# sbelharbi/sr-caco-2

Measured on AMD Instinct MI355X. Metric: train patches/sec, SwinIR x8 64->512 1ch, higher is better.
Workload: dtype f32 (fp16x2 split-MFMA, f32 accumulate)

## Files before the change

### include/srhip.h

```cpp
#ifndef SRHIP_H
#define SRHIP_H
#ifdef __cplusplus
extern "C" {
#endif
#if defined(__GNUC__) || defined(__clang__)
#pragma GCC visibility push(default)
#endif

const char* srhip_last_error(void);
int srhip_abi_version(void);
int srhip_experiments_enabled(void);
int srhip_set_matmul_mode(int mode);
int srhip_get_matmul_mode(void);


int srhip_gemm_nt(const float* A, long lda, const float* W, long ldw, const float* bias, float* C,
                  long ldc, int M, int N, int K, int a_mode, const float* ln_stats, int epi,
                  const float* R, long ldr, const float* rowscale, int rows_per_scale, float alpha,
                  float* aux, long ldaux, void* stream);

int srhip_gemm_nt_batched(const float* A, long lda, long a_z0, long a_z1, const float* W, long ldw, long w_z0, long w_z1, float* C,
                          long ldc, long c_z0, long c_z1, int M, int N, int K, int zcount, int zdiv, void* stream);

int srhip_conv3x3_nhwc(const float* X, long ldx, const float* Wp, const float* bias, float* Y, long ldy,
// ... 115 lines not shown
  float* part;
  float* part_colsum;
} srhip_tn_problem;
int srhip_tn_tiles(int NI, int NJ);
int srhip_tn_group_plan(int M, int ntiles, int* S);
int srhip_gemm_tn_grouped(const srhip_tn_problem* probs, int nprob, int M, int S, void* stream);
int srhip_conv3x3_wgrad(const float* dY, long lddy, const float* X, long ldx, int B, int H, int W,
                        int Cout, int Cin, float* part, float* part_colsum, int S, void* stream);

int srhip_tn_plan_bx3(int M, int NI, int NJ, int conv, int* S, long* part_floats);
int srhip_tn_group_plan_bx3(int M, int ntiles, int* S);
int srhip_gemm_tn_bx3(const float* A, long lda, const float* B, long ldb, int M, int NI, int NJ,
                      const float* a_rowscale, int a_rowscale_rows, int b_mode, const float* ln_stats,
                      float* part, float* part_colsum, int S, void* stream);
int srhip_gemm_tn_grouped_bx3(const srhip_tn_problem* probs, int nprob, int M, int S, void* stream);
int srhip_conv3x3_wgrad_bx3(const float* dY, long lddy, const float* X, long ldx, int B, int H, int W,
                            int Cout, int Cin, float* part, float* part_colsum, int S, void* stream);
int srhip_reduce_linear_wgrad(const float* part, const float* colsum, int S, float* dW, float* db,
                              int N, int K, void* stream);
long srhip_ln_affine_ws(int N, int K);
int srhip_reduce_ln_linear_wgrad(const float* part, const float* colsum, int S, const float* W,
                                 const float* gamma, const float* beta, float* dW, float* db,
                                 float* dgamma, float* dbeta, int N, int K, float* ln_ws,
                                 void* stream);
typedef struct {
  const float* part; const float* colsum;
  const float* W; const float* gamma; const float* beta;
  float* dW; float* db; float* dgamma; float* dbeta;
  int N, K;
  float* ln_ws;
} srhip_reduce_problem;
int srhip_reduce_wgrad_grouped(const srhip_reduce_problem* probs, int nprob, int S, void* stream);
int srhip_reduce_conv_wgrad(const float* part, const float* colsum, int S, float* dW, float* db,
                            int Co, int Ci, void* stream);

int srhip_fold_layernorm(const float* W, const float* b, const float* gamma, const float* beta,
                         float* Wf, float* bf, int N, int K, void* stream);
int srhip_transpose(const float* in, float* out, int R, int C, void* stream);
int srhip_pack_conv_weight(const float* w, float* wp, float* wpt, int Co, int Ci, void* stream);

int srhip_layernorm_fwd(const float* x, float* stats, float* y, const float* gamma, const float* beta,
                        long M, int C, void* stream);
long srhip_layernorm_bwd_ws(long M, int C);
int srhip_layernorm_bwd(const float* dy, const float* x, const float* stats, const float* res,
                        const float* gamma, float* out, float* dgamma, float* dbeta, float* workspace, long M,
                        int C, void* stream);

// ... 215 lines not shown
```

### sr-caco-2_amd/csrc/api.hip

```cpp
#include <stdarg.h>
#include "common.h"
#include "kernels.h"
#include "../../include/srhip.h"

static thread_local char g_err[512] = "";

int sr_fail(int code, const char* fmt, ...) {
  va_list ap;
  va_start(ap, fmt);
  vsnprintf(g_err, sizeof(g_err), fmt, ap);
  va_end(ap);
  return code;
}

extern "C" {

const char* srhip_last_error(void) { return g_err; }
int srhip_abi_version(void) { return 13; }
int srhip_experiments_enabled(void) {
#ifdef SRHIP_EXPERIMENTS
  return 1;
#else
  return 0;
#endif
// ... 357 lines not shown
}
int srhip_gemm_tn_bx3(const float* A, long lda, const float* B, long ldb, int M, int NI, int NJ,
                      const float* a_rowscale, int a_rowscale_rows, int b_mode, const float* ln_stats,
                      float* part, float* part_colsum, int S, void* stream) {
  return gemm_tn_any(true, A, lda, B, ldb, M, NI, NJ, a_rowscale, a_rowscale_rows, b_mode, ln_stats, part,
                     part_colsum, S, stream);
}

int srhip_tn_tiles(int NI, int NJ) { return sr_tn_tiles(NI, NJ); }
int srhip_tn_plan_bx3(int M, int NI, int NJ, int conv, int* S, long* part_floats) {
  return sr_tn_plan_bx3(M, NI, NJ, conv, S, part_floats);
}
int srhip_tn_group_plan_bx3(int M, int ntiles, int* S) { return sr_tn_group_plan_t(M, ntiles, 256, S); }
int srhip_tn_group_plan(int M, int ntiles, int* S) { return sr_tn_group_plan(M, ntiles, S); }

static int gemm_tn_grouped_any(bool bx, const srhip_tn_problem* probs, int nprob, int M, int S, void* stream) {
  SR_REQUIRE(nprob >= 1 && nprob <= (bx ? 24 : 4), "gemm_tn_grouped: 1..%d problems", bx ? 24 : 4);
  TnArgs a[24];
  memset(a, 0, sizeof(a));
  for (int k = 0; k < nprob; ++k) {
    const srhip_tn_problem& q = probs[k];
    SR_REQUIRE(q.b_mode >= 0 && q.b_mode <= 2, "gemm_tn_grouped: b_mode %d", q.b_mode);
    SR_REQUIRE(q.b_mode != 1 || q.ln_stats, "gemm_tn_grouped: layernorm prologue without stats");
    TnArgs& p = a[k];
    p.A = q.A; p.lda = q.lda; p.B = q.B; p.ldb = q.ldb; p.M = M; p.NI = q.NI; p.NJ = q.NJ;
    p.a_rowscale = q.a_rowscale; p.a_rowscale_rows = q.a_rowscale_rows; p.b_mode = q.b_mode;
    p.ln_stats = q.ln_stats; p.part = q.part; p.part_colsum = q.part_colsum; p.S = S;
  }
  return bx ? sr_gemm_tnb_grouped(a, nprob, (hipStream_t)stream) : sr_gemm_tn_grouped(a, nprob, (hipStream_t)stream);
}
int srhip_gemm_tn_grouped(const srhip_tn_problem* probs, int nprob, int M, int S, void* stream) {
  return gemm_tn_grouped_any(false, probs, nprob, M, S, stream);
}
int srhip_gemm_tn_grouped_bx3(const srhip_tn_problem* probs, int nprob, int M, int S, void* stream) {
  return gemm_tn_grouped_any(true, probs, nprob, M, S, stream);
}

static int conv3x3_ps2_split(int wfmt, const float* X, long ldx, const void* Wb, const float* bias, float* Yup, long ldy,
                          int B, int H, int W, int Cin, int Cout, int epi, float alpha, void* stream) {
  SR_REQUIRE(epi == 0 || epi == 1 || epi == 6, "conv3x3_ps2_bx3: epi %d (0 bias | 1 relu | 6 leaky relu)", epi);
  NtArgs p;
  memset(&p, 0, sizeof(p));
  p.A = X; p.lda = ldx; p.Wb = (const unsigned short*)Wb; p.C = Yup; p.ldc = ldy;
  p.N = Cout; p.K = Cin; p.bias = bias; p.epi = epi; p.rows_per_scale = H * W; p.alpha = alpha;
  p.batch = B; p.H = H; p.Wd = W; p.ps = 1; p.wfmt = wfmt;
  return sr_conv3x3_ntb(p, (hipStream_t)stream);
}
static int conv3x3_ps2_bwd_data_split(int wfmt, const float* dYup, long lddy, const void* Wbt, float* dX, long ldx, int B, int H,
                                   int W, int Cout, int Cin, int epi, const float* R, long ldr, float alpha,
                                   void* stream) {
// ... 56 lines not shown
```

### sr-caco-2_amd/csrc/gemm_tnb.hip

```cpp
#include <stdlib.h>
#include "common.h"
#include "kernels.h"

typedef __bf16 bf16x8 __attribute__((ext_vector_type(8)));
typedef __bf16 bf16x2 __attribute__((ext_vector_type(2)));
typedef float f32x2 __attribute__((ext_vector_type(2)));
typedef unsigned u32x4 __attribute__((ext_vector_type(4)));

namespace {

constexpr int TKB = 32;

__device__ const float k_tnb_zero_row[256] = {0.f};

__device__ __forceinline__ f32x16 mfma_bf(u32x4 a, u32x4 b, f32x16 c) {
  return __builtin_amdgcn_mfma_f32_32x32x16_bf16(__builtin_bit_cast(bf16x8, a),
                                                 __builtin_bit_cast(bf16x8, b), c, 0, 0, 0);
}

typedef _Float16 f16x8 __attribute__((ext_vector_type(8)));
typedef _Float16 tn_f16x2 __attribute__((ext_vector_type(2)));
__device__ __forceinline__ f32x16 mfma_h(u32x4 a, u32x4 b, f32x16 c) {
  return __builtin_amdgcn_mfma_f32_32x32x16_f16(__builtin_bit_cast(f16x8, a), __builtin_bit_cast(f16x8, b), c, 0, 0, 0);
}
// ... 315 lines not shown

  if (do_colsum) {
    float* red = (float*)smem;
    if (producer && !isB) {
#pragma unroll
      for (int j = 0; j < W; ++j) red[hh * BC + W * lane + j] = cs[j];
    }
    __syncthreads();
    if (tid < ivalid) {
      const int io = i0 + tid;
      p.part_colsum[(long)s * p.NI + (p.ps ? (io % ps_f) * 4 + io / ps_f : io)] = red[tid] + red[BC + tid];
    }
  }
}

template <int W, int BM = -1, bool AR = false, bool NR = false, bool CONV = false>
__device__ __forceinline__ void tnb_body_h(const TnArgs& p, const int s, const int tile, unsigned char* smem, const int tap = 0) {
  const int bmode = BM >= 0 ? BM : p.b_mode;
  const bool arow = BM >= 0 ? AR : (p.a_rowscale != nullptr);
  constexpr int BC = 64 * W, HC = 32 * W;
  constexpr int PLANE = 2 * BC * 64;
  constexpr int BUF = 3 * PLANE;
  constexpr int CTRL = 2 * PLANE;
  constexpr int SINV = 2 * PLANE + 4096;

  const int tid = threadIdx.x, lane = tid & 63;
  const int wave8 = __builtin_amdgcn_readfirstlane(tid >> 6);
  const bool producer = wave8 >= 4;
  const int wave = wave8 & 3;
  const int wi = wave >> 1, wj = wave & 1, r = lane & 31, h = lane >> 5;
  const int nbj = (p.NJ + p.j_tile - 1) / p.j_tile;
  const int bi = tile / nbj, bj = tile - bi * nbj;
  const int i0 = bi * p.i_tile, j0 = bj * p.j_tile;
  const int ivalid = min(p.i_tile, p.NI - i0), jvalid = min(p.j_tile, p.NJ - j0);
  const int m_begin = s * p.rows_per_slice;
  const int m_end = min(p.M, m_begin + p.rows_per_slice);
  const bool do_colsum = p.part_colsum && bj == 0 && tap == 0;
  const int cdy = CONV ? tap / 3 - 1 : 0, cdx = CONV ? tap % 3 - 1 : 0;

  struct Stage {
    typename ColVec<W>::T rv[2][8];
    float scale;
    float2 stats;
    int trow;
  };
  Stage sg0, sg1;
  const bool isB = wave & 1;
  const int ch = wave >> 1;
  const int lt = lane & 31, th = lane >> 5;
  const int opvalid = isB ? jvalid : ivalid;
  const int gcol = HC * ch + W * lt;
  const int colq = max(min(gcol, opvalid - W), 0);
  const int dsh = gcol - colq;
// ... 294 lines not shown
#pragma unroll
        for (int q = 0; q < 16; ++q) {
          const int row = (wi * W + i) * 32 + mfma_row(q, lane);
          if (row < ivalid) out[(long)(i0 + row) * p.NJ + j0 + col] = acc[i][j][q] * (sinv[row] * ib);
        }
      }
  }

  if (do_colsum) {
    float* red = (float*)smem;
    if (producer && !isB) {
#pragma unroll
      for (int j = 0; j < W; ++j) red[th * BC + gcol + j] = cs[j];
    }
    __syncthreads();
    if (tid < ivalid) p.part_colsum[(long)s * p.NI + i0 + tid] = red[tid] + red[BC + tid];
  }
}

constexpr int TK9 = 16;
__device__ __forceinline__ int unit_slot9(int col, int u) { return 2 * col + (u ^ ((col >> 3) & 1)); }
constexpr int T9_OPS = 6;
constexpr int T9_PLANE = T9_OPS * 64 * 32;
constexpr int T9_CTRL = 2 * T9_PLANE;
constexpr int T9_BUF = 2 * T9_PLANE + 2048;
constexpr int T9_SINV = 2 * T9_BUF;
constexpr int T9_LDS = 2 * T9_BUF + 2048;
constexpr int T9_THREADS = 14 * 64;

template <int H2, int DBG = 0>
// ... 513 lines not shown

template <int W>
__global__ void __launch_bounds__(512, 1) k_tnb_hc(TnArgs p, int tiles, int xcd) {
  extern __shared__ __attribute__((aligned(16))) unsigned char smem[];
  const int L = xcd ? sr_xcd_block(blockIdx.x, gridDim.x) : (int)blockIdx.x;
  const int tap = L % 9, t2 = L / 9;
  const bool even = p.NI % W == 0 && p.NJ % W == 0 && p.i_tile % W == 0 && p.j_tile % W == 0;
  if (even) tnb_body_h<W, 0, false, true, true>(p, t2 / tiles, t2 % tiles, smem, tap);
  else tnb_body_h<W, 0, false, false, true>(p, t2 / tiles, t2 % tiles, smem, tap);
}

constexpr int TNB_GROUP_MAX = 24;
struct TnbGroup {
  TnArgs p[TNB_GROUP_MAX];
  int tile_start[TNB_GROUP_MAX + 1];
  int n, S, xcd;
};
__device__ __forceinline__ void tnb_group_block(const TnbGroup& g, int& slice, int& t) {
  const int tiles = g.tile_start[g.n];
  if (g.xcd) {
    const int L = sr_xcd_block(blockIdx.x, gridDim.x);
    t = L % tiles;
    slice = L / tiles;
  } else {
    slice = blockIdx.x % g.S;
    t = blockIdx.x / g.S;
  }
}
template <int W>
__global__ void __launch_bounds__(512, 1) k_tnb_grouped(TnbGroup g) {
  extern __shared__ __attribute__((aligned(16))) unsigned char smem[];
  int slice, t;
  tnb_group_block(g, slice, t);
  TnArgs p = g.p[0];
  int t0 = 0;
#pragma unroll
  for (int i = 1; i < TNB_GROUP_MAX; ++i)
    if (i < g.n && t >= g.tile_start[i]) { p = g.p[i]; t0 = g.tile_start[i]; }
  tnb_body<W>(p, slice, t - t0, 0, smem);
}

template <int W>
__global__ void __launch_bounds__(512, 1) k_tnb_grouped_h(TnbGroup g) {
  extern __shared__ __attribute__((aligned(16))) unsigned char smem[];
  int slice, t;
  tnb_group_block(g, slice, t);
  TnArgs p = g.p[0];
  int t0 = 0;
#pragma unroll
  for (int i = 1; i < TNB_GROUP_MAX; ++i)
    if (i < g.n && t >= g.tile_start[i]) { p = g.p[i]; t0 = g.tile_start[i]; }
  const bool even = p.NI % W == 0 && p.NJ % W == 0 && p.i_tile % W == 0 && p.j_tile % W == 0;
  if (even && p.b_mode == 1 && !p.a_rowscale) tnb_body_h<W, 1, false, true>(p, slice, t - t0, smem);
  else if (even && p.b_mode == 0 && p.a_rowscale) tnb_body_h<W, 0, true, true>(p, slice, t - t0, smem);
  else if (even && p.b_mode == 2 && p.a_rowscale) tnb_body_h<W, 2, true, true>(p, slice, t - t0, smem);
  else tnb_body_h<W>(p, slice, t - t0, smem);
}

constexpr int TNB_BATCH_MAX = 40;
struct TnbConvBatch {
  TnArgs base;
  const float* A[TNB_BATCH_MAX];
  const float* B[TNB_BATCH_MAX];
  long part_stride, colsum_stride;
  int n, tiles, xcd;
};
template <int W>
__global__ void __launch_bounds__(512, 1) k_tnb_conv_batched(TnbConvBatch g) {
  extern __shared__ __attribute__((aligned(16))) unsigned char smem[];
  const int L = g.xcd ? sr_xcd_block(blockIdx.x, gridDim.x) : (int)blockIdx.x;
  const int tap = L % 9;
// ... 102 lines not shown
  if (e != hipSuccess) return sr_fail(-5, "%s: cannot reserve %d B of LDS: %s", name, bytes, hipGetErrorString(e));
  return 0;
}

constexpr int lds_bytes(int w) { return 2 * 3 * 2 * 64 * w * 64; }
constexpr long TNB_W1_SLOTS = 3 * 256;

}

int sr_gemm_tnb_grouped(TnArgs* probs, int n, hipStream_t st) {
  SR_REQUIRE(n >= 1 && n <= TNB_GROUP_MAX, "gemm_tn_grouped_bx3: 1..%d problems (got %d)", TNB_GROUP_MAX, n);
  static_assert(sizeof(TnbGroup) <= 4096, "kernel arguments");
  TnbGroup g;
  memset(&g, 0, sizeof(g));
  g.n = n;
  int w = 1, tiles = 0;
  for (int k = 0; k < n; ++k) {
    TnArgs& p = probs[k];
    SR_REQUIRE(p.M == probs[0].M && p.S == probs[0].S && !p.conv,
               "gemm_tn_grouped_bx3: problems must share M and S");
    SR_REQUIRE(p.NI % 4 == 0 && p.NJ % 4 == 0 && p.lda % 4 == 0 && p.ldb % 4 == 0,
               "gemm_tn_grouped_bx3: NI, NJ, lda, ldb must be multiples of 4");
    int a, b;
    p.i_tile = pick_tile(p.NI, &a);
    p.j_tile = pick_tile(p.NJ, &b);
    if (a > w) w = a;
    if (b > w) w = b;
    const int rps = sr_cdiv(p.M, p.S);
    p.rows_per_slice = (rps + TKB - 1) / TKB * TKB;
    g.tile_start[k] = tiles;
    tiles += sr_cdiv(p.NI, p.i_tile) * sr_cdiv(p.NJ, p.j_tile);
    g.p[k] = p;
  }
  g.tile_start[n] = tiles;
  g.S = probs[0].S;
  static const int gxcd = [] { const char* e = sr_getenv("SRHIP_TN_GROUP_XCD"); return e ? atoi(e) : 1; }();
  g.xcd = gxcd;
  dim3 grid(probs[0].S * tiles, 1, 1);
  static bool attr[4] = {false, false, false, false};
#define SR_TNB_G(W_)                                                                      \
  if (w == W_) {                                                                          \
    if (!attr[W_]) {                                                                      \
      if (int rc = reserve_lds(k_tnb_grouped<W_>, lds_bytes(W_), "k_tnb_grouped")) return rc; \
      attr[W_] = true;                                                                    \
    }                                                                                     \
    hipLaunchKernelGGL((k_tnb_grouped<W_>), grid, dim3(512), lds_bytes(W_), st, g);       \
  }
  if (w == 3) {
    static bool attr_h = false;
    if (!attr_h) {
      if (int rc = reserve_lds(k_tnb_grouped_h<3>, lds_bytes(3), "k_tnb_grouped_h")) return rc;
      attr_h = true;
    }
    hipLaunchKernelGGL((k_tnb_grouped_h<3>), grid, dim3(512), lds_bytes(3), st, g);
  }
  SR_TNB_G(1) SR_TNB_G(2)
#undef SR_TNB_G
  SR_LAUNCH_CHECK("k_tnb_grouped");
  return 0;
}

int sr_gemm_tnb(TnArgs& p, hipStream_t st) {
  SR_REQUIRE(p.M > 0 && p.S > 0, "gemm_tn_bx3: empty problem");
  SR_REQUIRE(p.NI % 4 == 0 && p.NJ % 4 == 0 && p.lda % 4 == 0 && p.ldb % 4 == 0,
             "gemm_tn_bx3: NI, NJ, lda, ldb must be multiples of 4");
  int tile;
  const int w = pick_w(p.NI, p.NJ, &tile);
  p.i_tile = p.j_tile = tile;
  SR_REQUIRE(!p.ps || (p.conv && p.NI % 4 == 0 && (p.NI / 4) % w == 0 && p.NI % p.i_tile == 0),
             "conv3x3_wgrad + PixelShuffle(2): Cout/4 = %d must be a multiple of %d (columns per lane), Cout of the tile", p.NI / 4, w);
  const int rps = sr_cdiv(p.M, p.S);
  p.rows_per_slice = (rps + TKB - 1) / TKB * TKB;
  int tiles = sr_cdiv(p.NI, p.i_tile) * sr_cdiv(p.NJ, p.j_tile);
// ... 174 lines not shown
```

### sr-caco-2_amd/csrc/kernels.h

```cpp
#pragma once
#include <hip/hip_runtime.h>

struct NtArgs {
  const float* A; long lda;
  const float* W; long ldw; long wtap;
  float* C; long ldc;
  int M, N, K;
  int n_tile;
  int xcd_order;
  const float* bias;
  int a_mode;
  const float* ln_stats;
  int epi;
  const float* slope;
  const float* pro_coef;
  const float* R; long ldr;
  float* aux; long ldaux;
  const float* R2; long ldr2; const float* ep_stats;
  int wide_epi;
  float* stats_out;
  const float* rowscale; int rows_per_scale; float alpha;
  int batch, H, Wd, tiles_x, tiles_y;
  int dbg;
  int stagger;
// ... 114 lines not shown
int sr_prep_table(const PrepEntry* tab_dev, int n, int total_blocks, hipStream_t st);
__host__ __device__ static inline int sr_kp(int K) { return (K + 31) / 32 * 32; }
int sr_split3(const float* W, long ldw, int rows, int K, unsigned short* out, hipStream_t st);
int sr_gemm_ntb(NtArgs& p, hipStream_t st);
int sr_conv3x3_ntb(NtArgs& p, hipStream_t st);
int sr_gemm_ntb_lnbwd(NtArgs& p, hipStream_t st);
int sr_gemm_ntp(NtArgs& p, hipStream_t st);
int sr_gemm_ntw(NtArgs& p, hipStream_t st);
int sr_conv3x3_ntcw(NtArgs& p, hipStream_t st);
int sr_conv3x3_ntcw2(NtArgs& p, int rows_per_wave, hipStream_t st);
int sr_conv3x3_nhcw(NtArgs& p, hipStream_t st);
int sr_conv3x3_nhcw2(NtArgs& p, int rows_per_wave, hipStream_t st);
int sr_gemm_tn(TnArgs& p, hipStream_t st);
int sr_gemm_tnb(TnArgs& p, hipStream_t st);
int sr_gemm_tnb_grouped(TnArgs* probs, int n, hipStream_t st);
int sr_tn_plan(int M, int NI, int NJ, int conv, int* S, long* part_floats);
int sr_gemm_tn_grouped(TnArgs* probs, int n, hipStream_t st);
int sr_tn_group_plan(int M, int ntiles, int* S);
int sr_tn_plan_t(int M, int NI, int NJ, int conv, int target, int* S, long* part_floats);
int sr_tn_plan_bx3(int M, int NI, int NJ, int conv, int* S, long* part_floats);
int sr_tn_group_plan_t(int M, int ntiles, int dflt_target, int* S);
int sr_tn_tiles(int NI, int NJ);
int sr_conv_wgrad_batched_plan(int n, int M, int NI, int NJ, int* S, long* part_floats_per_item);
int sr_conv_wgrad_batched_tnb(const TnArgs& base, const float* const* A, const float* const* B, int n,
                              long part_stride, long colsum_stride, hipStream_t st);
```

### sr-caco-2_amd/csrc/misc.hip

```cpp
#include "common.h"
#include "kernels.h"
#include "../../include/srhip.h"

namespace {

__global__ void k_reduce_slices(const float* __restrict__ part, float* __restrict__ out,
                                long n, int S, float beta, const float* __restrict__ colsum,
                                float* __restrict__ db, int nb, int main_blocks) {
  if ((int)blockIdx.x >= main_blocks) {
    const int j = (blockIdx.x - main_blocks) * blockDim.x + threadIdx.x;
    if (j < nb) {
      float d = 0.f;
      for (int s = 0; s < S; ++s) d += colsum[(long)s * nb + j];
      db[j] = d;
    }
    return;
  }
  for (long i = blockIdx.x * (long)blockDim.x + threadIdx.x; i < n;
       i += (long)main_blocks * blockDim.x) {
    float a = 0.f;
    int s = 0;
    for (; s + 8 <= S; s += 8) {
      float v[8];
#pragma unroll
// ... 140 lines not shown
    for (; rb < nrb; rb += 16) a0 += q[(long)rb * 2 * K];
  }
  sm[rl][c] = (a0 + a1) + (a2 + a3);
  __syncthreads();
  if (rl == 0 && idx < 2 * K) {
    float t = 0.f;
#pragma unroll
    for (int r = 0; r < 16; ++r) t += sm[r][c];
    (which ? dbeta : dgamma)[k] = t;
  }
}
struct ReduceGroup {
  struct P {
    const float* part; const float* colsum; const float* W; const float* gamma; const float* beta;
    float* dW; float* db; float* dgamma; float* dbeta; float* lnws;
    int N, K, blk0, kblocks, fblk0;
  } p[24];
  int n, S;
};
constexpr int RG_ROWS = 16;
__global__ void __launch_bounds__(256) k_reduce_group(ReduceGroup g) {
  __shared__ float sd[RG_ROWS], sg[4][64], sb[4][64];
  ReduceGroup::P P = g.p[0];
#pragma unroll
  for (int i = 1; i < 24; ++i)
    if (i < g.n && (int)blockIdx.x >= g.p[i].blk0) P = g.p[i];
  const int S = g.S, N = P.N, K = P.K;
  const int lb = blockIdx.x - P.blk0;
  const int bx = lb % P.kblocks, by = lb / P.kblocks;
  const int c = threadIdx.x & 63, rr = threadIdx.x >> 6;
  const int k = bx * 64 + c;
  if (threadIdx.x < RG_ROWS) {
    const int n = by * RG_ROWS + threadIdx.x;
    float d = 0.f;
    if (n < N)
      for (int s = 0; s < S; ++s) d += P.colsum[(long)s * N + n];
    sd[threadIdx.x] = d;
    if (n < N && bx == 0) P.db[n] = d;
  }
  __syncthreads();
  float ag = 0.f, ab = 0.f;
  const long sl = (long)N * K;
// ... 544 lines not shown
                                 const float* gamma, const float* beta, float* dW, float* db,
                                 float* dgamma, float* dbeta, int N, int K, float* ln_ws,
                                 void* stream) {
  hipStream_t st = (hipStream_t)stream;
  SR_REQUIRE(ln_ws != nullptr, "reduce_ln_linear_wgrad: workspace of srhip_ln_affine_ws(N, K) floats required");
  hipLaunchKernelGGL(k_fin_ln_linear, dim3(sr_cdiv(K, 64), sr_cdiv(N, 4)), dim3(256), 0, st, part,
                     colsum, S, W, gamma, beta, dW, db, ln_ws, N, K);
  hipLaunchKernelGGL(k_ln_affine_finish, dim3(sr_cdiv(2 * K, 256)), dim3(256), 0, st, ln_ws, sr_cdiv(N, 4), K,
                     dgamma, dbeta);
  SR_LAUNCH_CHECK("reduce_ln_linear_wgrad");
  return 0;
}

long srhip_ln_affine_ws(int N, int K) { return (long)sr_cdiv(N, 4) * 2 * K; }

int srhip_reduce_wgrad_grouped(const srhip_reduce_problem* probs, int nprob, int S, void* stream) {
  SR_REQUIRE(nprob >= 1 && nprob <= 24 && S > 0, "reduce_wgrad_grouped: 1..24 problems, S > 0");
  ReduceGroup g;
  memset(&g, 0, sizeof(g));
  g.n = nprob; g.S = S;
  int blocks = 0, fblocks = 0;
  for (int i = 0; i < nprob; ++i) {
    const srhip_reduce_problem& q = probs[i];
    SR_REQUIRE(q.part && q.colsum && q.dW && q.db && q.N > 0 && q.K > 0, "reduce_wgrad_grouped: problem %d incomplete", i);
    SR_REQUIRE(!q.gamma || (q.W && q.beta && q.dgamma && q.dbeta && q.ln_ws), "reduce_wgrad_grouped: LayerNorm problem %d incomplete", i);
    ReduceGroup::P& d = g.p[i];
    d.lnws = q.ln_ws;
    d.fblk0 = fblocks;
    if (q.gamma) fblocks += sr_cdiv(2 * q.K, 256);
    d.part = q.part; d.colsum = q.colsum; d.W = q.W; d.gamma = q.gamma; d.beta = q.beta;
    d.dW = q.dW; d.db = q.db; d.dgamma = q.dgamma; d.dbeta = q.dbeta; d.N = q.N; d.K = q.K;
    d.blk0 = blocks; d.kblocks = sr_cdiv(q.K, 64);
    blocks += d.kblocks * sr_cdiv(q.N, RG_ROWS);
  }
  hipLaunchKernelGGL(k_reduce_group, dim3(blocks), dim3(256), 0, (hipStream_t)stream, g);
  if (fblocks) hipLaunchKernelGGL(k_ln_affine_finish_group, dim3(fblocks), dim3(256), 0, (hipStream_t)stream, g);
  SR_LAUNCH_CHECK("reduce_wgrad_grouped");
  return 0;
}

int srhip_reduce_conv_wgrad(const float* part, const float* colsum, int S, float* dW, float* db,
                            int Co, int Ci, void* stream) {
  hipStream_t st = (hipStream_t)stream;
  const int mb = ew_grid((long)Co * Ci * 9);
  const bool bias = colsum && db;
  hipLaunchKernelGGL(k_reduce_conv_w, dim3(mb + (bias ? 1 : 0)), dim3(256), 0, st, part, dW, Co, Ci, S,
                     colsum, db, mb);
  SR_LAUNCH_CHECK("reduce_conv_wgrad");
  return 0;
}

int srhip_conv3x3_wgrad_batched_plan(int n, int B, int H, int W, int Cout, int Cin, int* S,
                                     long* part_floats_per_item) {
// ... 278 lines not shown
```

### sr-caco-2_amd/srhip/ops.py

```python
import ctypes

import torch

from . import probe
from ._lib import call, lib, SrhipError


def _chk(*ts):
    for t in ts:
        if t is None:
            continue
        if not t.is_cuda:
            raise SrhipError("srhip ops need CUDA/HIP tensors (no CPU fallback exists)")
        if t.dtype not in (torch.float32, torch.float64, torch.int32):
            raise SrhipError(f"unsupported dtype {t.dtype}")


def _p(t):
    return None if t is None else t.data_ptr()


def _st():
    return torch.cuda.current_stream().cuda_stream

# ... 1003 lines not shown
class _TnProblem(ctypes.Structure):
    _fields_ = [("A", ctypes.c_void_p), ("lda", ctypes.c_long), ("B", ctypes.c_void_p),
                ("ldb", ctypes.c_long), ("NI", ctypes.c_int), ("NJ", ctypes.c_int),
                ("a_rowscale", ctypes.c_void_p), ("a_rowscale_rows", ctypes.c_int),
                ("b_mode", ctypes.c_int), ("ln_stats", ctypes.c_void_p),
                ("part", ctypes.c_void_p), ("part_colsum", ctypes.c_void_p)]


class _ReduceProblem(ctypes.Structure):
    _fields_ = [("part", ctypes.c_void_p), ("colsum", ctypes.c_void_p), ("W", ctypes.c_void_p),
                ("gamma", ctypes.c_void_p), ("beta", ctypes.c_void_p), ("dW", ctypes.c_void_p),
                ("db", ctypes.c_void_p), ("dgamma", ctypes.c_void_p), ("dbeta", ctypes.c_void_p),
                ("N", ctypes.c_int), ("K", ctypes.c_int), ("ln_ws", ctypes.c_void_p)]


def linear_wgrad_grouped(problems):
    n = len(problems)
    M = problems[0]["dY"].shape[0]
    dev = problems[0]["dY"].device
    tiles = sum(lib.srhip_tn_tiles(q["dY"].shape[1], q["X"].shape[1]) for q in problems)
    S = ctypes.c_int(0)
    call("srhip_tn_group_plan" + _tn_sfx(), M, tiles, ctypes.addressof(S))
    S = S.value
    sizes = [(q["dY"].shape[1] * q["X"].shape[1], q["dY"].shape[1]) for q in problems]
    part = SCRATCH.get("tng_part", S * sum(a for a, _ in sizes), device=dev)
    cs = SCRATCH.get("tng_colsum", S * sum(b for _, b in sizes), device=dev)
    arr = (_TnProblem * n)()
    views = []
    po = co = 0
    for k, q in enumerate(problems):
        dY, X = q["dY"], q["X"]
        _chk(dY, X, q["dW"], q["db"], q.get("a_rowscale"), q.get("ln_stats"))
        N, K = dY.shape[1], X.shape[1]
        pk, ck = part[po:po + S * N * K], cs[co:co + S * N]
        po += S * N * K
        co += S * N
        views.append((pk, ck))
        a = arr[k]
        a.A, a.lda, a.B, a.ldb, a.NI, a.NJ = _p(dY), dY.stride(0), _p(X), X.stride(0), N, K
        a.a_rowscale, a.a_rowscale_rows = _p(q.get("a_rowscale")), q.get("a_rowscale_rows", 1)
        a.b_mode, a.ln_stats = q.get("b_mode", 0), _p(q.get("ln_stats"))
        a.part, a.part_colsum = _p(pk), _p(ck)
    if probe.on("linear_tn"):
        fl = sum(2.0 * M * q["dY"].shape[1] * q["X"].shape[1] for q in problems)
        by = sum(4.0 * (M * (q["dY"].shape[1] + q["X"].shape[1]) + q["dY"].shape[1] * q["X"].shape[1]) for q in problems)
        with probe.timed(("linear_tn", M, n), fl, by):
            call("srhip_gemm_tn_grouped" + _tn_sfx(), ctypes.addressof(arr), n, M, S, _st())
    else:
        call("srhip_gemm_tn_grouped" + _tn_sfx(), ctypes.addressof(arr), n, M, S, _st())
    red = (_ReduceProblem * n)()
    lnsz = [lib.srhip_ln_affine_ws(q["dY"].shape[1], q["X"].shape[1]) if q.get("ln") is not None else 0 for q in problems]
    lnws = SCRATCH.get("ln_affine_ws_g", max(1, sum(lnsz)), device=dev)
    lo = 0
    for r, q, (pk, ck), lsz in zip(red, problems, views, lnsz):
        r.part, r.colsum, r.dW, r.db = _p(pk), _p(ck), _p(q["dW"]), _p(q["db"])
        r.N, r.K = q["dY"].shape[1], q["X"].shape[1]
        if q.get("ln") is not None:
            W, gamma, beta, dgamma, dbeta = q["ln"]
            r.W, r.gamma, r.beta, r.dgamma, r.dbeta = _p(W), _p(gamma), _p(beta), _p(dgamma), _p(dbeta)
            r.ln_ws = _p(lnws[lo:lo + lsz])
            lo += lsz
    call("srhip_reduce_wgrad_grouped", ctypes.addressof(red), n, S, _st())


def ps2_fusable(Cin, Cout):
    return use_bx3() and Cout % 256 == 0 and Cin % 4 == 0 and Cin <= 128 and bx3_for(Cout, Cin) and bx3_nt_for(Cout, Cin)


def resblock64_fusable(F, Wp=None):
    return F == 64 and F16X2_CONV and (Wp is None or (isinstance(Wp, Bx3) and Wp.fmt == 1))


def resblock64_fwd(x, W1, b1, W2, b2, res_scale, a, out):
    _chk(x, b1, b2, a, out)
    B, H, W, C = x.shape
    assert C == 64 and a.shape == x.shape == out.shape and x.stride(3) == 1 and x.stride(1) == W * x.stride(2)
    assert all(isinstance(w, Bx3) and w.fmt == 1 and (w.rows, w.K) == (9 * 64, 64) for w in (W1, W2))
# ... 703 lines not shown
```

### sr-caco-2_amd/srhip/swinir_engine.py

```python
import os

import torch

from . import ops


class _Bufs:

    def __init__(self):
        self.d = {}

    def get(self, key, *shape, device="cuda", dtype=torch.float32):
        t = self.d.get(key)
        if t is None or tuple(t.shape) != tuple(shape) or t.dtype != dtype:
            if t is not None:
                ops.note_realloc()
            t = torch.empty(shape, device=device, dtype=dtype)
            self.d[key] = t
        return t

    def clear(self):
        if self.d:
            ops.note_realloc()
        self.d.clear()
# ... 560 lines not shown
                fn()
                done = torch.cuda.Event()
                done.record(self.wstream)
            return done

        dtn = buf("dtn", T, C)
        resi_conv_bwd("cab", "conv_after_body.", df, sv["tn"].view(B, H, W, C), sv["cab_rc"], dtn.view(B, H, W, C))
        dt = buf("dt", T, C)
        ops.layernorm_bwd(dtn, sv["t_last"], sv["st_n"], dt, gamma=net.norm.weight.data,
                          dgamma=G("norm.weight"), dbeta=G("norm.bias"))
        def layer_bufs(par):
            sfx = f".p{par}" if side_on else ""
            return ([buf(f"g{i}{sfx}", T, C) for i in range(2 * nset + 1)], [buf(f"dh{i}{sfx}", T, hid) for i in range(nset)],
                    [buf(f"dqkv{i}{sfx}", T, 3 * C) for i in range(nset)], sfx)
        gbufs, dhs, dqkvs, sfx = layer_bufs(0)
        recompute_gh = (self.fuse_mlp_h and ws.use_bx3 and ops.F16X2 and os.environ.get("SRHIP_RECOMPUTE_GH", "0") == "1")
        ghs = [None if recompute_gh else buf(f"gh{i}", T, hid) for i in range(nset)]
        ghs2 = [None if recompute_gh else buf(f"gh{i}.p1", T, hid) for i in range(nset)] if side_on else ghs
        dxh, da = buf("dxh", T, C), buf("da", T, C)
        nrot = len(gbufs)
        bi = len(self.blocks)
        dbT_all = buf("dbiasT_all", len(self.blocks), max(b.num_heads for b in self.blocks), 64, 64)
        for li in reversed(range(len(net.layers))):
            layer = net.layers[li]
            t_in, t_blocks, rc = sv["layers"][li]
            pre = f"layers.{li}."
            if side_on:
                gbufs, dhs, dqkvs, sfx = layer_bufs(li & 1)
                if len(side_done) >= 2:
                    main_stream.wait_event(side_done[-2])
            ghs_l = ghs2 if (side_on and (li & 1)) else ghs
# ... 131 lines not shown
```

Baseline: 728.9.

## Enable GELU recompute in wgrad by default with per-problem slice planning

Turns on recomputing the MLP GELU activation inside the fc2 weight-gradient GEMM producer by default, instead of reading a stored gh buffer. This saves the memory traffic of writing and reading that buffer. A specialised producer stage applies GELU and the row scale on the fly, and the grouped TN GEMM and the reduce kernels now accept a separate split-K slice count for each problem. A cost-weighted planner gives extra slices to the heavier GELU problems so blocks stay balanced. The cost is extra arithmetic in the producer and more complex block-index decoding.

Measured after the change: 730.9 (median of 5 runs). Within noise of the previous version (+0.3%).

```diff
diff --git a/include/srhip.h b/include/srhip.h
--- a/include/srhip.h
+++ b/include/srhip.h
@@ -153,6 +153,8 @@
                       const float* a_rowscale, int a_rowscale_rows, int b_mode, const float* ln_stats,
                       float* part, float* part_colsum, int S, void* stream);
 int srhip_gemm_tn_grouped_bx3(const srhip_tn_problem* probs, int nprob, int M, int S, void* stream);
+int srhip_tn_group_plan_pp_bx3(int M, int nprob, const int* tiles, const int* b_mode, int* S);
+int srhip_gemm_tn_grouped_pp_bx3(const srhip_tn_problem* probs, const int* S, int nprob, int M, void* stream);
 int srhip_conv3x3_wgrad_bx3(const float* dY, long lddy, const float* X, long ldx, int B, int H, int W,
                             int Cout, int Cin, float* part, float* part_colsum, int S, void* stream);
 int srhip_reduce_linear_wgrad(const float* part, const float* colsum, int S, float* dW, float* db,
@@ -170,6 +172,7 @@
   float* ln_ws;
 } srhip_reduce_problem;
 int srhip_reduce_wgrad_grouped(const srhip_reduce_problem* probs, int nprob, int S, void* stream);
+int srhip_reduce_wgrad_grouped_pp(const srhip_reduce_problem* probs, const int* S, int nprob, void* stream);
 int srhip_reduce_conv_wgrad(const float* part, const float* colsum, int S, float* dW, float* db,
                             int Co, int Ci, void* stream);
 
diff --git a/sr-caco-2_amd/csrc/api.hip b/sr-caco-2_amd/csrc/api.hip
--- a/sr-caco-2_amd/csrc/api.hip
+++ b/sr-caco-2_amd/csrc/api.hip
@@ -395,7 +395,7 @@
 int srhip_tn_group_plan_bx3(int M, int ntiles, int* S) { return sr_tn_group_plan_t(M, ntiles, 256, S); }
 int srhip_tn_group_plan(int M, int ntiles, int* S) { return sr_tn_group_plan(M, ntiles, S); }
 
-static int gemm_tn_grouped_any(bool bx, const srhip_tn_problem* probs, int nprob, int M, int S, void* stream) {
+static int gemm_tn_grouped_any(bool bx, const srhip_tn_problem* probs, int nprob, int M, int S, const int* Sk, void* stream) {
   SR_REQUIRE(nprob >= 1 && nprob <= (bx ? 24 : 4), "gemm_tn_grouped: 1..%d problems", bx ? 24 : 4);
   TnArgs a[24];
   memset(a, 0, sizeof(a));
@@ -406,15 +406,23 @@
     TnArgs& p = a[k];
     p.A = q.A; p.lda = q.lda; p.B = q.B; p.ldb = q.ldb; p.M = M; p.NI = q.NI; p.NJ = q.NJ;
     p.a_rowscale = q.a_rowscale; p.a_rowscale_rows = q.a_rowscale_rows; p.b_mode = q.b_mode;
-    p.ln_stats = q.ln_stats; p.part = q.part; p.part_colsum = q.part_colsum; p.S = S;
+    p.ln_stats = q.ln_stats; p.part = q.part; p.part_colsum = q.part_colsum; p.S = Sk ? Sk[k] : S;
   }
   return bx ? sr_gemm_tnb_grouped(a, nprob, (hipStream_t)stream) : sr_gemm_tn_grouped(a, nprob, (hipStream_t)stream);
 }
 int srhip_gemm_tn_grouped(const srhip_tn_problem* probs, int nprob, int M, int S, void* stream) {
-  return gemm_tn_grouped_any(false, probs, nprob, M, S, stream);
+  return gemm_tn_grouped_any(false, probs, nprob, M, S, nullptr, stream);
 }
 int srhip_gemm_tn_grouped_bx3(const srhip_tn_problem* probs, int nprob, int M, int S, void* stream) {
-  return gemm_tn_grouped_any(true, probs, nprob, M, S, stream);
+  return gemm_tn_grouped_any(true, probs, nprob, M, S, nullptr, stream);
+}
+int srhip_tn_group_plan_pp_bx3(int M, int nprob, const int* tiles, const int* b_mode, int* S) {
+  SR_REQUIRE(tiles && b_mode && S, "tn_group_plan_pp_bx3: null argument");
+  return sr_tn_group_plan_pp(M, nprob, tiles, b_mode, S);
+}
+int srhip_gemm_tn_grouped_pp_bx3(const srhip_tn_problem* probs, const int* S, int nprob, int M, void* stream) {
+  SR_REQUIRE(S, "gemm_tn_grouped_pp_bx3: slice counts required");
+  return gemm_tn_grouped_any(true, probs, nprob, M, 0, S, stream);
 }
 
 static int conv3x3_ps2_split(int wfmt, const float* X, long ldx, const void* Wb, const float* bias, float* Yup, long ldy,
diff --git a/sr-caco-2_amd/csrc/gemm_tnb.hip b/sr-caco-2_amd/csrc/gemm_tnb.hip
--- a/sr-caco-2_amd/csrc/gemm_tnb.hip
+++ b/sr-caco-2_amd/csrc/gemm_tnb.hip
@@ -353,8 +353,192 @@
   }
 }
 
+template <int W>
+__device__ __forceinline__ void tnb_stage_gh(const TnArgs& p, unsigned char* smem, const int wave, const int lane,
+                                             const int m_begin, const int m_end, const int i0, const int j0,
+                                             const int ivalid, const int jvalid, const bool do_colsum) {
+  constexpr int BC = 64 * W, QC = 16 * W;
+  constexpr int PLANE = 2 * BC * 64;
+  constexpr int BUF = 3 * PLANE;
+  constexpr int CTRL = 2 * PLANE;
+  constexpr int SINV = 2 * PLANE + 4096;
+  struct Stage {
+    typename ColVec<W>::T rv[2][8];
+    float scale;
+  };
+  Stage sg0, sg1;
+  const int lt = lane & 15;
+  const int oc = 2 * (lane >> 5) + ((((lt + 4) >> 3) ^ (lane >> 4)) & 1);
+  const int gcol = QC * wave + W * lt;
+  const int colA = max(min(gcol, ivalid - W), 0), colB = max(min(gcol, jvalid - W), 0);
+  const long ldA = p.lda, ldB = p.ldb;
+  const float* const pA = p.A + i0;
+  const float* const pB = p.B + j0;
+  const unsigned offA = (unsigned)((8L * oc * ldA + colA) * 4), offB = (unsigned)((8L * oc * ldB + colB) * 4);
+  float cs[W], sc[2][W];
+#pragma unroll
+  for (int j = 0; j < W; ++j) { cs[j] = 0.f; sc[0][j] = sc[1][j] = 0x1p126f; }
+
+  auto load = [&](int mc, Stage& sg) __attribute__((always_inline)) {
+    const int tokl = mc + (lane & 31);
+    const bool interior = mc + TKB <= m_end;
+    const bool tin = interior || tokl < m_end;
+    sg.scale = ldg_f(tin ? p.a_rowscale + tokl / p.a_rowscale_rows : k_sr_neutral + 1);
+    const float* qa = pA + (long)mc * ldA;
+    const float* qb = pB + (long)mc * ldB;
+#pragma unroll
+    for (int t = 0; t < 8; ++t) {
+      const bool ok = mc + 8 * oc + t < m_end;
+      sg.rv[0][t] = ColVec<W>::ldg(ok ? (const float*)((const char*)qa + offA) : k_tnb_zero_row);
+      qa += ldA;
+    }
+#pragma unroll
+    for (int t = 0; t < 8; ++t) {
+      const bool ok = mc + 8 * oc + t < m_end;
+      sg.rv[1][t] = ColVec<W>::ldg(ok ? (const float*)((const char*)qb + offB) : k_tnb_zero_row);
+      qb += ldB;
+    }
+  };
+  auto load_i = [&](int mc, Stage& sg) __attribute__((always_inline)) {
+    const int tokl = mc + (lane & 31);
+    sg.scale = ldg_f(p.a_rowscale + tokl / p.a_rowscale_rows);
+    const float* qa = pA + (long)mc * ldA;
+    const float* qb = pB + (long)mc * ldB;
+#pragma unroll
+    for (int t = 0; t < 8; ++t) {
+      sg.rv[0][t] = ColVec<W>::ldg(qa, offA);
+      qa += ldA;
+    }
+#pragma unroll
+    for (int t = 0; t < 8; ++t) {
+      sg.rv[1][t] = ColVec<W>::ldg(qb, offB);
+      qb += ldB;
+    }
+  };
+  auto bcast = [&](float v, int k) __attribute__((always_inline)) -> float {
+    const int vi = __builtin_bit_cast(int, v);
+    const int a0 = __builtin_amdgcn_readlane(vi, k), a1 = __builtin_amdgcn_readlane(vi, 8 + k);
+    const int a2 = __builtin_amdgcn_readlane(vi, 16 + k), a3 = __builtin_amdgcn_readlane(vi, 24 + k);
+    const int lo = (oc & 1) ? a1 : a0, hi = (oc & 1) ? a3 : a2;
+    return __builtin_bit_cast(float, (oc & 2) ? hi : lo);
+  };
+  auto store = [&](unsigned char* buf, const Stage& sg) {
+    sr_f32x2 x[2][4][W];
+#pragma unroll
+    for (int o = 0; o < 2; ++o)
+#pragma unroll
+      for (int t = 0; t < 4; ++t)
+#pragma unroll
+        for (int j = 0; j < W; ++j)
+          x[o][t][j] = sr_f32x2{ColVec<W>::at(sg.rv[o][2 * t], j), ColVec<W>::at(sg.rv[o][2 * t + 1], j)};
+#pragma unroll
+    for (int t = 0; t < 4; ++t) {
+      const float k0 = bcast(sg.scale, 2 * t), k1 = bcast(sg.scale, 2 * t + 1);
+#pragma unroll
+      for (int j = 0; j < W; ++j) { x[0][t][j].x *= k0; x[0][t][j].y *= k1; }
+    }
+    if (do_colsum) {
+#pragma unroll
+      for (int t = 0; t < 4; ++t)
+#pragma unroll
+        for (int j = 0; j < W; ++j) cs[j] += x[0][t][j].x + x[0][t][j].y;
+    }
+#pragma unroll
+    for (int t = 0; t < 4; ++t)
+#pragma unroll
+      for (int j = 0; j < W; ++j) x[1][t][j] = gelu_fast2(x[1][t][j]);
+    float f[2][W];
+    bool chg = false;
+#pragma unroll
+    for (int o = 0; o < 2; ++o)
+#pragma unroll
+      for (int j = 0; j < W; ++j) {
+        float mx = 0.f;
+#pragma unroll
+        for (int t = 0; t < 4; ++t) mx = fmaxf(mx, fmaxf(fabsf(x[o][t][j].x), fabsf(x[o][t][j].y)));
+        mx = fmaxf(mx, __shfl_xor(mx, 16));
+        mx = fmaxf(mx, __shfl_xor(mx, 32));
+        f[o][j] = 1.f;
+        if (mx * sc[o][j] > 60000.f) {
+          const float ns = exp2f(fminf(floorf(log2f(16384.f / mx)), 120.f));
+          f[o][j] = ns / sc[o][j];
+          sc[o][j] = ns;
+          chg = true;
+        }
+      }
+    const bool any = __any(chg);
+    float* ctrl = (float*)(buf + CTRL);
+    if (oc == 0) {
+#pragma unroll
+      for (int o = 0; o < 2; ++o)
+#pragma unroll
+        for (int j = 0; j < W; ++j) ctrl[o * BC + gcol + j] = f[o][j];
+    }
+    if (lane == 0) ((int*)(ctrl + 2 * BC))[wave] = any ? 1 : 0;
+#pragma unroll
+    for (int o = 0; o < 2; ++o)
+#pragma unroll
+      for (int j = 0; j < W; ++j) {
+        unsigned qh[4], ql[4];
+#pragma unroll
+        for (int t = 0; t < 4; ++t) split2_pair(x[o][t][j].x * sc[o][j], x[o][t][j].y * sc[o][j], qh[t], ql[t]);
+        unsigned char* dst = buf + unit_slot<W>(o * BC + gcol + j, oc) * 16;
+        *(u32x4*)(dst) = u32x4{qh[0], qh[1], qh[2], qh[3]};
+        *(u32x4*)(dst + PLANE) = u32x4{ql[0], ql[1], ql[2], ql[3]};
+      }
+  };
+
+  const int nch = ((m_end - m_begin + 2 * TKB - 1) / (2 * TKB)) * 2;
+  __builtin_amdgcn_s_setprio(2);
+  const int n_int = (m_end - m_begin) / TKB;
+  int c = 0;
+  if (n_int >= 5) {
+    load_i(m_begin, sg0);
+    load_i(m_begin + TKB, sg1);
+    store(smem, sg0);
+    load_i(m_begin + 2 * TKB, sg0);
+    __syncthreads();
+    for (; c + 4 < n_int; c += 2) {
+      store(smem + BUF, sg1);
+      load_i(m_begin + (c + 3) * TKB, sg1);
+      __syncthreads();
+      store(smem, sg0);
+      load_i(m_begin + (c + 4) * TKB, sg0);
+      __syncthreads();
+    }
+  } else {
+    load(m_begin, sg0);
+    load(m_begin + TKB, sg1);
+    store(smem, sg0);
+    load(m_begin + 2 * TKB, sg0);
+    __syncthreads();
+  }
+  for (; c < nch; c += 2) {
+    store(smem + BUF, sg1);
+    load(m_begin + (c + 3) * TKB, sg1);
+    __syncthreads();
+    store(smem, sg0);
+    load(m_begin + (c + 4) * TKB, sg0);
+    __syncthreads();
+  }
+  if (oc == 0) {
+#pragma unroll
+    for (int o = 0; o < 2; ++o)
+#pragma unroll
+      for (int j = 0; j < W; ++j) ((float*)(smem + SINV))[o * BC + gcol + j] = 1.0f / sc[o][j];
+  }
+  __syncthreads();
+  if (do_colsum) {
+    float* red = (float*)smem;
+#pragma unroll
+    for (int j = 0; j < W; ++j) red[oc * BC + gcol + j] = cs[j];
+    __syncthreads();
+  }
+}
+
 template <int W, int BM = -1, bool AR = false, bool NR = false, bool CONV = false>
 __device__ __forceinline__ void tnb_body_h(const TnArgs& p, const int s, const int tile, unsigned char* smem, const int tap = 0) {
+  constexpr bool QCUT = BM == 2 && AR && NR && !CONV;
   const int bmode = BM >= 0 ? BM : p.b_mode;
   const bool arow = BM >= 0 ? AR : (p.a_rowscale != nullptr);
   constexpr int BC = 64 * W, HC = 32 * W;
@@ -376,6 +560,12 @@
   const int m_end = min(p.M, m_begin + p.rows_per_slice);
   const bool do_colsum = p.part_colsum && bj == 0 && tap == 0;
   const int cdy = CONV ? tap / 3 - 1 : 0, cdx = CONV ? tap % 3 - 1 : 0;
+  if constexpr (QCUT) {
+    if (producer) {
+      tnb_stage_gh<W>(p, smem, wave, lane, m_begin, m_end, i0, j0, ivalid, jvalid, do_colsum);
+      return;
+    }
+  }
 
   struct Stage {
     typename ColVec<W>::T rv[2][8];
@@ -700,6 +890,10 @@
       for (int j = 0; j < W; ++j) red[th * BC + gcol + j] = cs[j];
     }
     __syncthreads();
+    if constexpr (QCUT) {
+      if (tid < ivalid) p.part_colsum[(long)s * p.NI + i0 + tid] = (red[tid] + red[BC + tid]) + (red[2 * BC + tid] + red[3 * BC + tid]);
+      return;
+    }
     if (tid < ivalid) p.part_colsum[(long)s * p.NI + i0 + tid] = red[tid] + red[BC + tid];
   }
 }
@@ -1243,47 +1437,48 @@
 struct TnbGroup {
   TnArgs p[TNB_GROUP_MAX];
   int tile_start[TNB_GROUP_MAX + 1];
+  int blk_start[TNB_GROUP_MAX + 1];
   int n, S, xcd;
+  int tiles;
 };
-__device__ __forceinline__ void tnb_group_block(const TnbGroup& g, int& slice, int& t) {
-  const int tiles = g.tile_start[g.n];
-  if (g.xcd) {
-    const int L = sr_xcd_block(blockIdx.x, gridDim.x);
-    t = L % tiles;
-    slice = L / tiles;
-  } else {
-    slice = blockIdx.x % g.S;
-    t = blockIdx.x / g.S;
-  }
+__device__ __forceinline__ void tnb_group_block(const TnbGroup& g, TnArgs& p, int& slice, int& t) {
+  const int tiles = g.tiles;
+  const int L = g.xcd ? sr_xcd_block(blockIdx.x, gridDim.x) : (int)blockIdx.x;
+  int key = L;
+  if (g.S) {
+    if (g.xcd) { key = L % tiles; slice = L / tiles; }
+    else { slice = L % g.S; key = L / g.S; }
+  }
+  p = g.p[0];
+  int k0 = 0, nt = g.tile_start[1];
+#pragma unroll
+  for (int i = 1; i < TNB_GROUP_MAX; ++i) {
+    const int st = g.S ? g.tile_start[i] : g.blk_start[i];
+    if (i < g.n && key >= st) { p = g.p[i]; k0 = st; nt = g.tile_start[i + 1] - g.tile_start[i]; }
+  }
+  t = key - k0;
+  if (!g.S) { slice = t / nt; t -= slice * nt; }
 }
 template <int W>
 __global__ void __launch_bounds__(512, 1) k_tnb_grouped(TnbGroup g) {
   extern __shared__ __attribute__((aligned(16))) unsigned char smem[];
   int slice, t;
-  tnb_group_block(g, slice, t);
-  TnArgs p = g.p[0];
-  int t0 = 0;
-#pragma unroll
-  for (int i = 1; i < TNB_GROUP_MAX; ++i)
-    if (i < g.n && t >= g.tile_start[i]) { p = g.p[i]; t0 = g.tile_start[i]; }
-  tnb_body<W>(p, slice, t - t0, 0, smem);
+  TnArgs p;
+  tnb_group_block(g, p, slice, t);
+  tnb_body<W>(p, slice, t, 0, smem);
 }
 
 template <int W>
 __global__ void __launch_bounds__(512, 1) k_tnb_grouped_h(TnbGroup g) {
   extern __shared__ __attribute__((aligned(16))) unsigned char smem[];
   int slice, t;
-  tnb_group_block(g, slice, t);
-  TnArgs p = g.p[0];
-  int t0 = 0;
-#pragma unroll
-  for (int i = 1; i < TNB_GROUP_MAX; ++i)
-    if (i < g.n && t >= g.tile_start[i]) { p = g.p[i]; t0 = g.tile_start[i]; }
+  TnArgs p;
+  tnb_group_block(g, p, slice, t);
   const bool even = p.NI % W == 0 && p.NJ % W == 0 && p.i_tile % W == 0 && p.j_tile % W == 0;
-  if (even && p.b_mode == 1 && !p.a_rowscale) tnb_body_h<W, 1, false, true>(p, slice, t - t0, smem);
-  else if (even && p.b_mode == 0 && p.a_rowscale) tnb_body_h<W, 0, true, true>(p, slice, t - t0, smem);
-  else if (even && p.b_mode == 2 && p.a_rowscale) tnb_body_h<W, 2, true, true>(p, slice, t - t0, smem);
-  else tnb_body_h<W>(p, slice, t - t0, smem);
+  if (even && p.b_mode == 1 && !p.a_rowscale) tnb_body_h<W, 1, false, true>(p, slice, t, smem);
+  else if (even && p.b_mode == 0 && p.a_rowscale) tnb_body_h<W, 0, true, true>(p, slice, t, smem);
+  else if (even && p.b_mode == 2 && p.a_rowscale) tnb_body_h<W, 2, true, true>(p, slice, t, smem);
+  else tnb_body_h<W>(p, slice, t, smem);
 }
 
 constexpr int TNB_BATCH_MAX = 40;
@@ -1416,13 +1611,14 @@
   TnbGroup g;
   memset(&g, 0, sizeof(g));
   g.n = n;
-  int w = 1, tiles = 0;
+  int w = 1, tiles = 0, blocks = 0;
+  bool one_s = true;
   for (int k = 0; k < n; ++k) {
     TnArgs& p = probs[k];
-    SR_REQUIRE(p.M == probs[0].M && p.S == probs[0].S && !p.conv,
-               "gemm_tn_grouped_bx3: problems must share M and S");
+    SR_REQUIRE(p.M == probs[0].M && p.S >= 1 && !p.conv, "gemm_tn_grouped_bx3: problems must share M; S >= 1");
     SR_REQUIRE(p.NI % 4 == 0 && p.NJ % 4 == 0 && p.lda % 4 == 0 && p.ldb % 4 == 0,
                "gemm_tn_grouped_bx3: NI, NJ, lda, ldb must be multiples of 4");
+    one_s = one_s && p.S == probs[0].S;
     int a, b;
     p.i_tile = pick_tile(p.NI, &a);
     p.j_tile = pick_tile(p.NJ, &b);
@@ -1431,14 +1627,18 @@
     const int rps = sr_cdiv(p.M, p.S);
     p.rows_per_slice = (rps + TKB - 1) / TKB * TKB;
     g.tile_start[k] = tiles;
-    tiles += sr_cdiv(p.NI, p.i_tile) * sr_cdiv(p.NJ, p.j_tile);
+    g.blk_start[k] = blocks;
+    const int nt = sr_cdiv(p.NI, p.i_tile) * sr_cdiv(p.NJ, p.j_tile);
+    tiles += nt;
+    blocks += nt * p.S;
     g.p[k] = p;
   }
-  g.tile_start[n] = tiles;
-  g.S = probs[0].S;
+  g.tile_start[n] = g.tiles = tiles;
+  g.blk_start[n] = blocks;
+  g.S = one_s ? probs[0].S : 0;
   static const int gxcd = [] { const char* e = sr_getenv("SRHIP_TN_GROUP_XCD"); return e ? atoi(e) : 1; }();
   g.xcd = gxcd;
-  dim3 grid(probs[0].S * tiles, 1, 1);
+  dim3 grid(blocks, 1, 1);
   static bool attr[4] = {false, false, false, false};
 #define SR_TNB_G(W_)                                                                      \
   if (w == W_) {                                                                          \
@@ -1459,6 +1659,36 @@
   SR_TNB_G(1) SR_TNB_G(2)
 #undef SR_TNB_G
   SR_LAUNCH_CHECK("k_tnb_grouped");
+  return 0;
+}
+
+constexpr float TNB_COST_GELU = 1.15f;
+int sr_tn_group_plan_pp(int M, int n, const int* tiles, const int* b_mode, int* S) {
+  SR_REQUIRE(n >= 1 && n <= TNB_GROUP_MAX, "tn_group_plan_pp_bx3: 1..%d problems (got %d)", TNB_GROUP_MAX, n);
+  int tot = 0;
+  for (int k = 0; k < n; ++k) {
+    SR_REQUIRE(tiles[k] >= 1, "tn_group_plan_pp_bx3: problem %d has no tiles", k);
+    tot += tiles[k];
+  }
+  int s0;
+  if (int rc = sr_tn_group_plan_t(M, tot, 256, &s0)) return rc;
+  for (int k = 0; k < n; ++k) S[k] = s0;
+  const int smax = min((M + 127) / 128, 256);
+  long blocks = (long)tot * s0;
+  for (;;) {
+    float worst = 0.f;
+    for (int k = 0; k < n; ++k) worst = fmaxf(worst, (b_mode[k] == 2 ? TNB_COST_GELU : 1.f) / (float)S[k]);
+    int need = 0, most = 0;
+    for (int k = 0; k < n; ++k)
+      if ((b_mode[k] == 2 ? TNB_COST_GELU : 1.f) / (float)S[k] >= worst * (1.f - 1e-6f)) {
+        need += tiles[k];
+        most = max(most, S[k]);
+      }
+    if (need == tot || blocks + need > 256 || most + 1 > smax) break;
+    for (int k = 0; k < n; ++k)
+      if ((b_mode[k] == 2 ? TNB_COST_GELU : 1.f) / (float)S[k] >= worst * (1.f - 1e-6f)) ++S[k];
+    blocks += need;
+  }
   return 0;
 }
 
diff --git a/sr-caco-2_amd/csrc/kernels.h b/sr-caco-2_amd/csrc/kernels.h
--- a/sr-caco-2_amd/csrc/kernels.h
+++ b/sr-caco-2_amd/csrc/kernels.h
@@ -152,6 +152,7 @@
 int sr_gemm_tn(TnArgs& p, hipStream_t st);
 int sr_gemm_tnb(TnArgs& p, hipStream_t st);
 int sr_gemm_tnb_grouped(TnArgs* probs, int n, hipStream_t st);
+int sr_tn_group_plan_pp(int M, int n, const int* tiles, const int* b_mode, int* S);
 int sr_tn_plan(int M, int NI, int NJ, int conv, int* S, long* part_floats);
 int sr_gemm_tn_grouped(TnArgs* probs, int n, hipStream_t st);
 int sr_tn_group_plan(int M, int ntiles, int* S);
diff --git a/sr-caco-2_amd/csrc/misc.hip b/sr-caco-2_amd/csrc/misc.hip
--- a/sr-caco-2_amd/csrc/misc.hip
+++ b/sr-caco-2_amd/csrc/misc.hip
@@ -178,9 +178,9 @@
   struct P {
     const float* part; const float* colsum; const float* W; const float* gamma; const float* beta;
     float* dW; float* db; float* dgamma; float* dbeta; float* lnws;
-    int N, K, blk0, kblocks, fblk0;
+    int N, K, S, blk0, kblocks, fblk0;
   } p[24];
-  int n, S;
+  int n;
 };
 constexpr int RG_ROWS = 16;
 __global__ void __launch_bounds__(256) k_reduce_group(ReduceGroup g) {
@@ -189,7 +189,7 @@
 #pragma unroll
   for (int i = 1; i < 24; ++i)
     if (i < g.n && (int)blockIdx.x >= g.p[i].blk0) P = g.p[i];
-  const int S = g.S, N = P.N, K = P.K;
+  const int S = P.S, N = P.N, K = P.K;
   const int lb = blockIdx.x - P.blk0;
   const int bx = lb % P.kblocks, by = lb / P.kblocks;
   const int c = threadIdx.x & 63, rr = threadIdx.x >> 6;
@@ -764,17 +764,19 @@
 
 long srhip_ln_affine_ws(int N, int K) { return (long)sr_cdiv(N, 4) * 2 * K; }
 
-int srhip_reduce_wgrad_grouped(const srhip_reduce_problem* probs, int nprob, int S, void* stream) {
-  SR_REQUIRE(nprob >= 1 && nprob <= 24 && S > 0, "reduce_wgrad_grouped: 1..24 problems, S > 0");
+static int reduce_wgrad_grouped_any(const srhip_reduce_problem* probs, int nprob, int S, const int* Sk, void* stream) {
+  SR_REQUIRE(nprob >= 1 && nprob <= 24, "reduce_wgrad_grouped: 1..24 problems");
   ReduceGroup g;
   memset(&g, 0, sizeof(g));
-  g.n = nprob; g.S = S;
+  g.n = nprob;
   int blocks = 0, fblocks = 0;
   for (int i = 0; i < nprob; ++i) {
     const srhip_reduce_problem& q = probs[i];
     SR_REQUIRE(q.part && q.colsum && q.dW && q.db && q.N > 0 && q.K > 0, "reduce_wgrad_grouped: problem %d incomplete", i);
     SR_REQUIRE(!q.gamma || (q.W && q.beta && q.dgamma && q.dbeta && q.ln_ws), "reduce_wgrad_grouped: LayerNorm problem %d incomplete", i);
     ReduceGroup::P& d = g.p[i];
+    d.S = Sk ? Sk[i] : S;
+    SR_REQUIRE(d.S > 0, "reduce_wgrad_grouped: problem %d: S > 0", i);
     d.lnws = q.ln_ws;
     d.fblk0 = fblocks;
     if (q.gamma) fblocks += sr_cdiv(2 * q.K, 256);
@@ -787,6 +789,14 @@
   if (fblocks) hipLaunchKernelGGL(k_ln_affine_finish_group, dim3(fblocks), dim3(256), 0, (hipStream_t)stream, g);
   SR_LAUNCH_CHECK("reduce_wgrad_grouped");
   return 0;
+}
+int srhip_reduce_wgrad_grouped(const srhip_reduce_problem* probs, int nprob, int S, void* stream) {
+  SR_REQUIRE(S > 0, "reduce_wgrad_grouped: 1..24 problems, S > 0");
+  return reduce_wgrad_grouped_any(probs, nprob, S, nullptr, stream);
+}
+int srhip_reduce_wgrad_grouped_pp(const srhip_reduce_problem* probs, const int* S, int nprob, void* stream) {
+  SR_REQUIRE(S, "reduce_wgrad_grouped_pp: slice counts required");
+  return reduce_wgrad_grouped_any(probs, nprob, 0, S, stream);
 }
 
 int srhip_reduce_conv_wgrad(const float* part, const float* colsum, int S, float* dW, float* db,
diff --git a/sr-caco-2_amd/srhip/ops.py b/sr-caco-2_amd/srhip/ops.py
--- a/sr-caco-2_amd/srhip/ops.py
+++ b/sr-caco-2_amd/srhip/ops.py
@@ -1041,17 +1041,27 @@
                 ("N", ctypes.c_int), ("K", ctypes.c_int), ("ln_ws", ctypes.c_void_p)]
 
 
-def linear_wgrad_grouped(problems):
+def linear_wgrad_grouped(problems, slices=None):
     n = len(problems)
     M = problems[0]["dY"].shape[0]
     dev = problems[0]["dY"].device
-    tiles = sum(lib.srhip_tn_tiles(q["dY"].shape[1], q["X"].shape[1]) for q in problems)
-    S = ctypes.c_int(0)
-    call("srhip_tn_group_plan" + _tn_sfx(), M, tiles, ctypes.addressof(S))
-    S = S.value
+    pp = _tn_sfx() == "_bx3"
+    ntile = [lib.srhip_tn_tiles(q["dY"].shape[1], q["X"].shape[1]) for q in problems]
+    if slices is not None:
+        assert pp and len(slices) == n
+        Sk = (ctypes.c_int * n)(*slices)
+        S = list(Sk)
+    elif pp:
+        Sk, tk, bk = (ctypes.c_int * n)(), (ctypes.c_int * n)(*ntile), (ctypes.c_int * n)(*[q.get("b_mode", 0) for q in problems])
+        call("srhip_tn_group_plan_pp_bx3", M, n, ctypes.addressof(tk), ctypes.addressof(bk), ctypes.addressof(Sk))
+        S = list(Sk)
+    else:
+        S1 = ctypes.c_int(0)
+        call("srhip_tn_group_plan" + _tn_sfx(), M, sum(ntile), ctypes.addressof(S1))
+        S = [S1.value] * n
     sizes = [(q["dY"].shape[1] * q["X"].shape[1], q["dY"].shape[1]) for q in problems]
-    part = SCRATCH.get("tng_part", S * sum(a for a, _ in sizes), device=dev)
-    cs = SCRATCH.get("tng_colsum", S * sum(b for _, b in sizes), device=dev)
+    part = SCRATCH.get("tng_part", sum(s * a for s, (a, _) in zip(S, sizes)), device=dev)
+    cs = SCRATCH.get("tng_colsum", sum(s * b for s, (_, b) in zip(S, sizes)), device=dev)
     arr = (_TnProblem * n)()
     views = []
     po = co = 0
@@ -1059,22 +1069,28 @@
         dY, X = q["dY"], q["X"]
         _chk(dY, X, q["dW"], q["db"], q.get("a_rowscale"), q.get("ln_stats"))
         N, K = dY.shape[1], X.shape[1]
-        pk, ck = part[po:po + S * N * K], cs[co:co + S * N]
-        po += S * N * K
-        co += S * N
+        pk, ck = part[po:po + S[k] * N * K], cs[co:co + S[k] * N]
+        po += S[k] * N * K
+        co += S[k] * N
         views.append((pk, ck))
         a = arr[k]
         a.A, a.lda, a.B, a.ldb, a.NI, a.NJ = _p(dY), dY.stride(0), _p(X), X.stride(0), N, K
         a.a_rowscale, a.a_rowscale_rows = _p(q.get("a_rowscale")), q.get("a_rowscale_rows", 1)
         a.b_mode, a.ln_stats = q.get("b_mode", 0), _p(q.get("ln_stats"))
         a.part, a.part_colsum = _p(pk), _p(ck)
+
+    def launch():
+        if pp:
+            call("srhip_gemm_tn_grouped_pp_bx3", ctypes.addressof(arr), ctypes.addressof(Sk), n, M, _st())
+        else:
+            call("srhip_gemm_tn_grouped" + _tn_sfx(), ctypes.addressof(arr), n, M, S[0], _st())
     if probe.on("linear_tn"):
         fl = sum(2.0 * M * q["dY"].shape[1] * q["X"].shape[1] for q in problems)
         by = sum(4.0 * (M * (q["dY"].shape[1] + q["X"].shape[1]) + q["dY"].shape[1] * q["X"].shape[1]) for q in problems)
         with probe.timed(("linear_tn", M, n), fl, by):
-            call("srhip_gemm_tn_grouped" + _tn_sfx(), ctypes.addressof(arr), n, M, S, _st())
-    else:
-        call("srhip_gemm_tn_grouped" + _tn_sfx(), ctypes.addressof(arr), n, M, S, _st())
+            launch()
+    else:
+        launch()
     red = (_ReduceProblem * n)()
     lnsz = [lib.srhip_ln_affine_ws(q["dY"].shape[1], q["X"].shape[1]) if q.get("ln") is not None else 0 for q in problems]
     lnws = SCRATCH.get("ln_affine_ws_g", max(1, sum(lnsz)), device=dev)
@@ -1087,7 +1103,10 @@
             r.W, r.gamma, r.beta, r.dgamma, r.dbeta = _p(W), _p(gamma), _p(beta), _p(dgamma), _p(dbeta)
             r.ln_ws = _p(lnws[lo:lo + lsz])
             lo += lsz
-    call("srhip_reduce_wgrad_grouped", ctypes.addressof(red), n, S, _st())
+    if pp:
+        call("srhip_reduce_wgrad_grouped_pp", ctypes.addressof(red), ctypes.addressof(Sk), n, _st())
+    else:
+        call("srhip_reduce_wgrad_grouped", ctypes.addressof(red), n, S[0], _st())
 
 
 def ps2_fusable(Cin, Cout):
diff --git a/sr-caco-2_amd/srhip/swinir_engine.py b/sr-caco-2_amd/srhip/swinir_engine.py
--- a/sr-caco-2_amd/srhip/swinir_engine.py
+++ b/sr-caco-2_amd/srhip/swinir_engine.py
@@ -598,7 +598,7 @@
             return ([buf(f"g{i}{sfx}", T, C) for i in range(2 * nset + 1)], [buf(f"dh{i}{sfx}", T, hid) for i in range(nset)],
                     [buf(f"dqkv{i}{sfx}", T, 3 * C) for i in range(nset)], sfx)
         gbufs, dhs, dqkvs, sfx = layer_bufs(0)
-        recompute_gh = (self.fuse_mlp_h and ws.use_bx3 and ops.F16X2 and os.environ.get("SRHIP_RECOMPUTE_GH", "0") == "1")
+        recompute_gh = (self.fuse_mlp_h and ws.use_bx3 and ops.F16X2 and os.environ.get("SRHIP_RECOMPUTE_GH", "1") != "0")
         ghs = [None if recompute_gh else buf(f"gh{i}", T, hid) for i in range(nset)]
         ghs2 = [None if recompute_gh else buf(f"gh{i}.p1", T, hid) for i in range(nset)] if side_on else ghs
         dxh, da = buf("dxh", T, C), buf("da", T, C)
```
